# devitocodes/seigen

Hardware: AMD Instinct MI355X
Metric: M DoF-updates/sec, 3D elastic P=4 (higher is better)
Workload: dtype f64

## Files before the change

### seigen_amd/csrc/kernels_mfma.hip

```cpp
#include <hip/hip_runtime.h>

#include "kernels.hpp"

namespace sg {

template <typename R>
struct RT;
template <>
struct RT<double> {
  typedef double v4 __attribute__((ext_vector_type(4)));
  static constexpr bool SMALL = true;
  static __device__ __forceinline__ v4 big(double a, double b, v4 c) { return __builtin_amdgcn_mfma_f64_16x16x4f64(a, b, c, 0, 0, 0); }
  static __device__ __forceinline__ double small(double a, double b, double c) { return __builtin_amdgcn_mfma_f64_4x4x4f64(a, b, c, 0, 0, 0); }
};
template <>
struct RT<float> {
  typedef float v4 __attribute__((ext_vector_type(4)));
  static constexpr bool SMALL = false;
  static __device__ __forceinline__ v4 big(float a, float b, v4 c) { return __builtin_amdgcn_mfma_f32_16x16x4f32(a, b, c, 0, 0, 0); }
  static __device__ __forceinline__ float small(float, float, float c) { return c; }
};

template <typename R, int P>
constexpr int mfma_resident_blocks() {
  return sizeof(R) == 4 ? 3 : (P == 1 ? 4 : (P == 2 ? 3 : 2));
}

template <int P, typename R>
struct MG {
  static constexpr int ND = ElemDims<3, P>::ND;
  static constexpr int NF = ElemDims<3, P>::NF;
  static constexpr int KS = (ND + 3) / 4;
  static constexpr int KSF = (NF + 3) / 4;
  static constexpr int MTF = RT<R>::SMALL ? ND / 16 : (ND + 15) / 16;
  static constexpr int NSM = RT<R>::SMALL ? (ND % 16 + 3) / 4 : 0;
  static constexpr int MTT = MTF + NSM;
  static constexpr int MTFA = MTF > 0 ? MTF : 1;
  static constexpr int NSMA = NSM > 0 ? NSM : 1;
  static constexpr int S4 = (ND + 3) / 4;
  static constexpr int NFRAG_F = MTT * 3 * KS;
  static constexpr int NFRAG_G = 3 * MTT * KS;
  static constexpr int NFRAG_L = 4 * MTT * KSF;
  static constexpr int RK = (P >= 2) ? ElemDims<3, (P >= 2 ? P - 1 : 1)>::ND : 1;
  static constexpr int QLT = RK / 16;
  static constexpr int QST = (RK % 16 + 3) / 4;
  static constexpr int KR = (RK + 3) / 4;
  static constexpr int NFRAG_Q = (QLT + QST) * KS;
  static constexpr int NFRAG_P = 3 * MTT * KR;
};

template <typename R, int P, int FACT>
constexpr bool g_stash() {
  return sizeof(R) == 8 && P == 4 && FACT == 1;
}
template <int NOUT, int LT, int ST, int NKS>
struct CompactTiles {
  static constexpr int NL = NOUT * LT * NKS * 64, NS = NOUT * ST * NKS * 16, N = NL + NS;
  static constexpr int at(int o, int t, int ks) {
    return t < LT ? ((o * LT + t) * NKS + ks) * 64 : NL + ((o * ST + (t - LT)) * NKS + ks) * 16;
  }
};
constexpr int G_STASH_SLOTS = 36;
constexpr int G_STASH_WAVES = 8;
template <typename R, int P, int STASH>
struct GLds {
  using M = MG<P, R>;
  static constexpr int STW = 3 * G_STASH_SLOTS * 16;
  static constexpr int OFF_FO = ((int)sizeof(MeshDev) + 15) / 16 * 16;
  static constexpr int OFF_AV = OFF_FO + (STASH ? 64 * (int)sizeof(int) : 0);
  static constexpr int OFF_Q = OFF_AV + (int)sizeof(R) * (STASH ? CompactTiles<3, M::MTF, M::NSM, M::KR>::N : M::NFRAG_P * 64);
  static constexpr int OFF_AL = OFF_Q + (int)sizeof(R) * (STASH ? CompactTiles<1, M::QLT, M::QST, M::KS>::N : M::NFRAG_Q * 64);
  static constexpr int OFF_ST = OFF_AL + (int)sizeof(R) * (STASH ? CompactTiles<4, M::MTF, M::NSM, M::KSF>::N : M::NFRAG_L * 64);
  static constexpr int BYTES = OFF_ST + (STASH ? G_STASH_WAVES * STW * (int)sizeof(R) : 0);
};

#define LD_STREAM(p) __builtin_nontemporal_load(p)
#define ST_STREAM(p, v) __builtin_nontemporal_store((v), (p))
#define SG_PRIO(p) __builtin_amdgcn_s_setprio(p)
constexpr int SG_PRIO_F0 = 0x120, SG_PRIO_F1 = 0x320, SG_PRIO_F2 = 0x320, SG_PRIO_G0 = 0x120, SG_PRIO_G1 = 0x120;
#define SG_PRIO_VOL ((PRIO3 >> 8) & 3)
#define SG_PRIO_LIFT ((PRIO3 >> 4) & 3)
#define SG_PRIO_EPI (PRIO3 & 3)
#define MFMA64(a, b, c) RT<R>::big((a), (b), (c))
#define MFMA4(a, b, c) RT<R>::small((a), (b), (c))

#ifdef SG_STAMPS
#define STAMP(t)                                                                   \
  do {                                                                             \
    __builtin_amdgcn_sched_barrier(0);                                             \
    asm volatile("s_memtime %0\n\ts_waitcnt lgkmcnt(0)" : "=s"(t)::"memory");       \
    __builtin_amdgcn_sched_barrier(0);                                             \
  } while (0)
#define STAMP_DECL unsigned long long st0 = 0, st1 = 0, st2 = 0, st3 = 0, st4 = 0, sta = 0, stb = 0, sacc[4] = {0, 0, 0, 0}, ssub[3] = {0, 0, 0}, sitems = 0
#define STAMP_ACC                                                                  \
  do {                                                                             \
    sacc[0] += st1 - st0;                                                          \
    sacc[1] += st2 - st1;                                                          \
    sacc[2] += st3 - st2;                                                          \
    sacc[3] += st4 - st3;                                                          \
    if (sta) { ssub[0] += sta - st2; ssub[1] += stb - sta; ssub[2] += st3 - stb; } \
    sitems += 1;                                                                   \
  } while (0)
#define STAMP_FLUSH                                                                \
  do {                                                                             \
    if (A.dbg && lane == 0) {                                                      \
      for (int z = 0; z < 4; ++z) atomicAdd(&A.dbg[z], sacc[z]);                   \
      atomicAdd(&A.dbg[4], sitems);                                                \
      for (int z = 0; z < 3; ++z) atomicAdd(&A.dbg[5 + z], ssub[z]);               \
    }                                                                              \
  } while (0)
#else
#define STAMP(t) do { } while (0)
#define STAMP_DECL
#define STAMP_ACC do { } while (0)
#define STAMP_FLUSH do { } while (0)
#endif

template <int SYM, typename R>
__device__ __forceinline__ void load_tensor(const R* p, int stride, R (&T)[9]) {
  if (SYM) {
    T[0] = p[0];
    T[1] = p[1 * stride];
    T[2] = p[2 * stride];
    T[4] = p[4 * stride];
    T[5] = p[5 * stride];
    T[8] = p[8 * stride];
    T[3] = T[1];
    T[6] = T[2];
    T[7] = T[5];
  } else {
#pragma unroll
    for (int c = 0; c < 9; ++c) T[c] = p[c * stride];
  }
}
__device__ __forceinline__ constexpr bool upper(int ij) { return (ij / 3) <= (ij % 3); }

template <int SYM, int GHOST, typename R>
__device__ __forceinline__ void load_trace(const bool cube_face, const R* p, bool ghost, const int (&tl)[6], R (&T)[6]) {
  if (cube_face) {
    if (SYM) {
#pragma unroll
      for (int i = 0; i < 3; ++i) T[i] = p[GHOST ? (ghost ? i : tl[i]) : tl[i]];
    } else {
      const R* pa = p + ((GHOST && ghost) ? 0 : tl[0]);
#pragma unroll
      for (int i = 0; i < 3; ++i) T[i] = pa[GHOST ? (ghost ? i : i * 48) : i * 48];
    }
  } else if (SYM) {
    T[0] = p[0];
    T[1] = p[1 * 16];
    T[2] = p[2 * 16];
    T[3] = p[4 * 16];
    T[4] = p[5 * 16];
    T[5] = p[8 * 16];
  } else {
    const R *pa = p + tl[0], *pb = p + tl[3];
#pragma unroll
    for (int i = 0; i < 3; ++i) {
      T[i] = pa[i * 48];
      T[3 + i] = pb[i * 48];
    }
  }
}

__device__ __forceinline__ bool uniform_nonzero(double c) {
  return (__builtin_bit_cast(unsigned long long, c) << 1) != 0ull;
}
__device__ __forceinline__ bool uniform_nonzero(float c) { return (__builtin_bit_cast(unsigned, c) << 1) != 0u; }

struct LaneGeo {
  long c;
  int cc[3];
  bool valid;
  bool active;
};

typedef __attribute__((address_space(4))) const MfmaConst cMfmaConst;
typedef __attribute__((address_space(4))) const MfmaClassConst cMfmaClassConst;

template <typename MD>
__device__ __forceinline__ LaneGeo lane_geo(const MD& md, const StageArgs& A, long g, int w) {
  LaneGeo L;
  L.c = g * 16 + w;
  L.valid = L.c < md.ncube;
  const unsigned cl = L.valid ? (unsigned)L.c : 0u;
  const unsigned n0 = (unsigned)md.n[0], n1 = (unsigned)md.n[1];
  const unsigned t = cl / n0, z = t / n1;
  L.cc[0] = (int)(cl - t * n0);
  L.cc[1] = (int)(t - z * n1);
  L.cc[2] = (int)z;
  bool in = false;
  for (int bx = 0; bx < A.nbox; ++bx) {
    bool ib = true;
#pragma unroll
    for (int a = 0; a < 3; ++a) ib = ib && (L.cc[a] >= A.boxes_o[bx][a]) && (L.cc[a] < A.boxes_o[bx][a] + A.boxes_n[bx][a]);
    in = in || ib;
  }
  L.active = L.valid && in;
  return L;
}

template <typename R>
struct NbrRef {
  const R* p;
  int cstride;
  bool ghost;
  bool physical;
};

__device__ __forceinline__ LaneGeo lane_geo_all(long ncube, long g, int w) {
  LaneGeo L;
  L.c = g * 16 + w;
  L.valid = L.c < ncube;
  L.cc[0] = L.cc[1] = L.cc[2] = 0;
  L.active = L.valid;
  return L;
}

typedef int nbr4 __attribute__((ext_vector_type(4)));
__device__ __forceinline__ nbr4 load_nbr4(const StageArgs& A, long item, int w) {
  return *reinterpret_cast<const nbr4*>(A.nbr_tab + (item * 16 + w) * 4);
}
template <int ND, int NF, int NC, typename R_>
__device__ __forceinline__ NbrRef<R_> nbr_from_entry(const StageArgs& A, int e, int side, const R_* own_base) {
  NbrRef<R_> R;
  const R_* const fin = reinterpret_cast<const R_*>(A.in);
  R.cstride = 16;
  R.ghost = e < -1;
  R.physical = e == -1;
  const long slot = e < 0 ? 0 : e;
  const R_* pin = fin + ((slot >> 4) * (long)ND) * NC * 16 + (slot & 15);
  R.p = e < 0 ? own_base : pin;
  if (__any(R.ghost)) {
    if (R.ghost) {
      R.p = reinterpret_cast<const R_*>(A.ghost[side]) + (long)(-2 - e) * NF * 3;
      R.cstride = 1;
    }
  }
  return R;
}

struct ItemRange {
  long lo, hi, step;
  long chunk, xcd, nitems;
};
__device__ __forceinline__ ItemRange item_range(long nitems, int wave, int spread, long chunk) {
  ItemRange r;
  const long wpb = blockDim.x >> 6;
  r.chunk = 0;
  r.xcd = 0;
  r.nitems = nitems;
  if (spread) {
    r.lo = (long)blockIdx.x * wpb + wave;
    r.hi = nitems;
    r.step = (long)gridDim.x * wpb;
    return r;
  }
  const long nblk = gridDim.x;
  const long xcd = blockIdx.x % 8;
  const long slot = blockIdx.x / 8;
  const long blocks_here = (nblk - xcd + 7) / 8;
  r.step = blocks_here * wpb;
  if (chunk > 0) {
    const long nchunks = (nitems + chunk - 1) / chunk;
    const long mine = (nchunks - xcd + 7) / 8;
    r.chunk = chunk;
    r.xcd = xcd;
    r.lo = slot * wpb + wave;
    r.hi = mine > 0 ? mine * chunk : 0;
    return r;
  }
  const long ipx = (nitems + 7) / 8;
  r.lo = xcd * ipx + slot * wpb + wave;
  r.hi = (xcd + 1) * ipx < nitems ? (xcd + 1) * ipx : nitems;
  return r;
}
__device__ __forceinline__ long item_of(const ItemRange& r, long it) {
  if (r.chunk == 0) return it;
  const long c = it / r.chunk;
  const long item = (c * 8 + r.xcd) * r.chunk + (it - c * r.chunk);
  return item < r.nitems ? item : -1;
}

template <int N, typename R, int NT = 256>
__device__ __forceinline__ void copy_to_lds(R* dst, const R* __restrict__ src) {
  constexpr int PER = (N + NT - 1) / NT;
  R v[PER];
#pragma unroll
  for (int j = 0; j < PER; ++j) {
    const int i = threadIdx.x + j * NT;
    v[j] = (i < N) ? src[i] : R(0);
  }
#pragma unroll
  for (int j = 0; j < PER; ++j) {
    const int i = threadIdx.x + j * NT;
    if (i < N) dst[i] = v[j];
  }
}

template <typename CT, int NOUT, int LT, int ST, int NKS, typename R, int NT>
__device__ __forceinline__ void copy_compact(R* dst, const R* __restrict__ src) {
  constexpr int PER = (CT::N + NT - 1) / NT;
  R v[PER];
#pragma unroll
  for (int j = 0; j < PER; ++j) {
    const int i = threadIdx.x + j * NT;
    int s = 0;
    if (i < CT::NL) {
      const int fr = i >> 6, o = fr / (LT * NKS), rem = fr - o * (LT * NKS);
      s = (o * (LT + ST) * NKS + rem) * 64 + (i & 63);
    } else {
      const int i2 = i - CT::NL, fr = i2 >> 4, c = i2 & 15, o = fr / (ST * NKS), rem = fr - o * (ST * NKS);
      s = (o * (LT + ST) * NKS + LT * NKS + rem) * 64 + (c & 3) + 16 * (c >> 2);
    }
    v[j] = (i < CT::N) ? src[s] : R(0);
  }
#pragma unroll
  for (int j = 0; j < PER; ++j) {
    const int i = threadIdx.x + j * NT;
    if (i < CT::N) dst[i] = v[j];
  }
}

template <int NV, int NL, typename R, int NT = 256>
__device__ __forceinline__ void load_tables(R* sAV, R* sAL, const StageArgs& A) {
  copy_to_lds<NV * 64, R, NT>(sAV, reinterpret_cast<const R*>(A.fragV));
  copy_to_lds<NL * 64, R, NT>(sAL, reinterpret_cast<const R*>(A.fragL));
  __syncthreads();
}

template <int NV, int NL, typename R>
__device__ __forceinline__ void load_tables(R* sAV, R* sAL, MeshDev* sMd, const StageArgs& A) {
  const int* src = reinterpret_cast<const int*>(A.md);
  int* dst = reinterpret_cast<int*>(sMd);
  constexpr int NI = (int)(sizeof(MeshDev) / sizeof(int)), PERI = (NI + 255) / 256;
  int w[PERI];
#pragma unroll
  for (int j = 0; j < PERI; ++j) {
    const int i = threadIdx.x + j * 256;
    w[j] = (i < NI) ? src[i] : 0;
  }
  copy_to_lds<NV * 64>(sAV, reinterpret_cast<const R*>(A.fragV));
  copy_to_lds<NL * 64>(sAL, reinterpret_cast<const R*>(A.fragL));
#pragma unroll
  for (int j = 0; j < PERI; ++j) {
    const int i = threadIdx.x + j * 256;
    if (i < NI) dst[i] = w[j];
  }
  __syncthreads();
}


template <typename R>
__device__ __forceinline__ R ndot(R c0, R c1, R c2, R t0, R t1, R t2) {
  R r = c0 * t0;
  r = __builtin_fma(c1, t1, r);
  r = __builtin_fma(c2, t2, r);
  return r;
}
template <>
__device__ __forceinline__ float ndot<float>(float c0, float c1, float c2, float t0, float t1, float t2) {
  float r = c0 * t0;
  r = __builtin_fmaf(c1, t1, r);
  r = __builtin_fmaf(c2, t2, r);
  return r;
}
__device__ __forceinline__ double fma_of(double a, double b, double c) { return __builtin_fma(a, b, c); }
__device__ __forceinline__ float fma_of(float a, float b, float c) { return __builtin_fmaf(a, b, c); }

template <int SYM, typename R>
__device__ __forceinline__ R trace_flux(const bool cube_face, int i, R wf, const R (&cnf)[3], const R (&tc)[2], const R (&T)[6]) {
  if (cube_face) return wf * (tc[0] * T[i]);
  if (SYM) {
    const int s0 = i, s1 = i == 0 ? 1 : (i == 1 ? 3 : 4), s2 = i == 0 ? 2 : (i == 1 ? 4 : 5);
    return wf * ndot<R>(cnf[0], cnf[1], cnf[2], T[s0], T[s1], T[s2]);
  }
  const R r = tc[0] * T[i];
  return wf * fma_of(tc[1], T[3 + i], r);
}


template <typename R, int P, int MODE, int SYM, bool FACT, bool STASH, bool DYN>
__device__ __forceinline__ void stage_G_body(const StageArgs& A) {
  using M = MG<P, R>;
  constexpr int NT = STASH ? 512 : 256;
  typedef typename RT<R>::v4 d4;
  constexpr int PRIO3 = MODE ? SG_PRIO_G1 : SG_PRIO_G0;
  constexpr int ND = M::ND, NF = M::NF, KS = M::KS, KSF = M::KSF, MTF = M::MTF, NSM = M::NSM, MTT = M::MTT, S4 = M::S4;
  constexpr int PF = sizeof(R) == 4 ? 6 : 4;
  constexpr int QLT = M::QLT, QST = M::QST, KR = M::KR;
  using CP = CompactTiles<3, MTF, NSM, KR>;
  using CQ = CompactTiles<1, QLT, QST, KS>;
  using CL = CompactTiles<4, MTF, NSM, KSF>;
  using LY = GLds<R, P, STASH>;
  constexpr int STW = LY::STW;
  R *sAV = nullptr, *sQ = nullptr, *sAL = nullptr, *sSt = nullptr;
  MeshDev* sMdp = nullptr;
  int* sFo = nullptr;
  if constexpr (DYN) {
    extern __shared__ __attribute__((aligned(16))) unsigned char sg_dyn_lds[];
    sMdp = reinterpret_cast<MeshDev*>(sg_dyn_lds);
    sFo = reinterpret_cast<int*>(sg_dyn_lds + LY::OFF_FO);
    sAV = reinterpret_cast<R*>(sg_dyn_lds + LY::OFF_AV);
    sQ = reinterpret_cast<R*>(sg_dyn_lds + LY::OFF_Q);
    sAL = reinterpret_cast<R*>(sg_dyn_lds + LY::OFF_AL);
    sSt = reinterpret_cast<R*>(sg_dyn_lds + LY::OFF_ST);
  } else {
    __shared__ R sAV_[(FACT ? M::NFRAG_P : M::NFRAG_G) * 64];
    __shared__ R sQ_[FACT ? M::NFRAG_Q * 64 : 1];
    __shared__ R sAL_[M::NFRAG_L * 64];
    __shared__ MeshDev sMd_;
    sAV = sAV_, sQ = sQ_, sAL = sAL_, sMdp = &sMd_;
  }
  MeshDev& sMd = *sMdp;
  if constexpr (STASH) {
    static_assert(ND <= G_STASH_SLOTS && 4 * KS <= G_STASH_SLOTS, "a stash slot per B row of the Q pass");
    copy_to_lds<(int)(sizeof(MeshDev) / sizeof(int)), int, NT>(reinterpret_cast<int*>(&sMd), reinterpret_cast<const int*>(A.md));
    copy_compact<CQ, 1, QLT, QST, KS, R, NT>(sQ, reinterpret_cast<const R*>(A.fragQ));
    copy_compact<CP, 3, MTF, NSM, KR, R, NT>(sAV, reinterpret_cast<const R*>(A.fragV));
    copy_compact<CL, 4, MTF, NSM, KSF, R, NT>(sAL, reinterpret_cast<const R*>(A.fragL));
    if (threadIdx.x < 64) {
      const int f = threadIdx.x >> 4, bq4 = 4 * (threadIdx.x & 3) + ((threadIdx.x >> 2) & 3);
      sFo[threadIdx.x] = (int)A.md->fnode[f][bq4 < NF ? bq4 : 0] * 16 * (int)sizeof(R);
    }
    __syncthreads();
  } else {
    if constexpr (FACT) copy_to_lds<M::NFRAG_Q * 64>(sQ, reinterpret_cast<const R*>(A.fragQ));
    load_tables<(FACT ? M::NFRAG_P : M::NFRAG_G), M::NFRAG_L>(sAV, sAL, &sMd, A);
  }

  const int lane = threadIdx.x & 63;
  const int wave = __builtin_amdgcn_readfirstlane(threadIdx.x >> 6);
  const int q = lane >> 4, w = lane & 15;
  typedef __attribute__((address_space(4))) const MeshDev cMeshDev;
  const cMeshDev* md = (const cMeshDev*)(unsigned long long)A.md;
  const R* __restrict__ in = reinterpret_cast<const R*>(A.in);
  R* __restrict__ out = reinterpret_cast<R*>(A.out);
  const R c_self = (R)A.c_self, c_new = (R)A.c_new;
  const long ngroups = sMd.ncube_pad >> 4;
  const ItemRange ir = item_range(A.item_list ? (long)A.nlist : ngroups * 6, wave, A.spread, A.order_chunk);

  STAMP_DECL;
  for (long it = ir.lo; it < ir.hi; it += ir.step) {
    STAMP(st0);
    const long iti = item_of(ir, it);
    if (iti < 0) continue;
    const long item = A.item_list ? (long)A.item_list[iti] : iti;
    const long g = item / 6;
    const int k = (int)(item - g * 6);
    const LaneGeo L = A.all_active ? lane_geo_all(sMd.ncube, g, w) : lane_geo(sMd, A, g, w);
    const nbr4 nbe = load_nbr4(A, item, w);
    if (!__any(L.active)) continue;
    const R* own = in + ((g * 6 + k) * (long)ND) * 3 * 16 + w;
    int qo = q * 3 * 16;
    asm volatile("" : "+v"(qo));
    const R* ownq = own + qo;
    const R* ownl = (4 * (KS - 1) + q < ND) ? ownq + (KS - 1) * 4 * 3 * 16 : own;
    auto brow = [&](int ks) { return (ks == KS - 1) ? ownl : ownq + ks * 4 * 3 * 16; };
    int lo = lane;
    asm volatile("" : "+v"(lo));
    const int lo4 = (lo & 3) + ((lo >> 4) << 2);
    R* const stw = sSt + (STASH ? wave * STW : 0) + lo;
    const char* const str = reinterpret_cast<const char*>(sSt + (STASH ? wave * STW : 0) + (lo & 15));
    auto tile = [&](const R* tab, int full, int at, int t, int nlarge) { return STASH ? tab[at + (t < nlarge ? lo : lo4)] : tab[full * 64 + lo]; };

    R Jm[3][3], cnf[4][3];
#pragma unroll
    for (int r = 0; r < 3; ++r)
#pragma unroll
      for (int j = 0; j < 3; ++j) Jm[r][j] = (R)(-md->Jinv[k][r][j]);
#pragma unroll
    for (int f = 0; f < 4; ++f)
#pragma unroll
      for (int j = 0; j < 3; ++j) cnf[f][j] = (R)md->cn[k][f][j];

    R Sd[3][S4], So[3][S4];
#pragma unroll
    for (int i = 0; i < 3; ++i)
#pragma unroll
      for (int m = 0; m < S4; ++m) Sd[i][m] = So[i][m] = R(0);

    constexpr int NB = 2;
    constexpr int NBO = (FACT && !STASH) ? NB : 1;
    R nx[NB][KSF][3], nxo[NBO][KSF][3];
    auto request = [&](int f, R (&dst)[KSF][3], R (&dso)[KSF][3]) {
      const NbrRef<R> NR = nbr_from_entry<ND, NF, 3>(A, nbe[f], 2 * sMd.nb_axis[k][f] + (sMd.nb_dir[k][f] > 0 ? 1 : 0), own);
#pragma unroll
      for (int ks = 0; ks < KSF; ++ks) {
        const int bb = (4 * ks + q < NF) ? 4 * ks + q : 0;
        const int on = sMd.fnode[f][bb];
        const int nn = NR.ghost ? sMd.nb_fnode[k][f][bb] : (NR.physical ? on : sMd.nb_node[k][f][bb]);
#pragma unroll
        for (int i = 0; i < 3; ++i) {
          dst[ks][i] = NR.p[(nn * 3 + i) * NR.cstride];
          if constexpr (FACT && !STASH) dso[ks][i] = own[(on * 3 + i) * 16];
        }
      }
    };
    SG_PRIO(SG_PRIO_VOL);
    STAMP(st1);
    auto fold_dir = [&](int r, const d4 (&acc)[M::MTFA][3], const R (&accs)[M::NSMA][3]) {
#pragma unroll
      for (int kk = 0; kk < 3; ++kk) {
        const R c = Jm[r][kk];
        if (uniform_nonzero(c)) {
#pragma unroll
          for (int i = 0; i < 3; ++i) {
#pragma unroll
            for (int t = 0; t < MTF; ++t)
#pragma unroll
              for (int reg = 0; reg < 4; ++reg) {
                if (4 * t + reg >= S4) continue;
                if (i == kk)
                  Sd[i][4 * t + reg] += c * acc[t][i][reg];
                else
                  So[i + kk - 1][4 * t + reg] += c * acc[t][i][reg];
              }
#pragma unroll
            for (int t = 0; t < NSM; ++t) {
              if (i == kk)
                Sd[i][4 * MTF + t] += c * accs[t][i];
              else
                So[i + kk - 1][4 * MTF + t] += c * accs[t][i];
            }
          }
        }
      }
#pragma unroll
      for (int m = 0; m < S4; ++m)
#pragma unroll
        for (int i = 0; i < 3; ++i) asm volatile("" : "+v"(Sd[i][m]), "+v"(So[i][m]));
    };
    auto tiles_step = [&](int nks, int r, int ks, const R (&b)[3], d4 (&acc)[M::MTFA][3], R (&accs)[M::NSMA][3]) {
#pragma unroll
      for (int t = 0; t < MTT; ++t) {
        const R a = tile(sAV, (r * MTT + t) * nks + ks, CP::at(r, t, ks), t, MTF);
#pragma unroll
        for (int i = 0; i < 3; ++i) {
          if (t < MTF)
            acc[t < MTF ? t : 0][i] = MFMA64(a, b[i], acc[t < MTF ? t : 0][i]);
          else
            accs[t < MTF ? 0 : t - MTF][i] = MFMA4(a, b[i], accs[t < MTF ? 0 : t - MTF][i]);
        }
      }
    };
    auto clear_acc = [&](d4 (&acc)[M::MTFA][3], R (&accs)[M::NSMA][3]) {
#pragma unroll
      for (int i = 0; i < 3; ++i) {
#pragma unroll
        for (int t = 0; t < MTF; ++t) acc[t][i] = d4{0, 0, 0, 0};
#pragma unroll
        for (int t = 0; t < NSM; ++t) accs[t][i] = R(0);
      }
    };
    if constexpr (!FACT) {
      constexpr int NS = 3 * KS;
      R bq[PF][3];
#pragma unroll
      for (int s = 0; s < PF; ++s)
#pragma unroll
        for (int i = 0; i < 3; ++i) bq[s][i] = brow(s % KS)[i * 16];
#pragma unroll
      for (int r = 0; r < 3; ++r) {
        d4 acc[M::MTFA][3];
        R accs[M::NSMA][3];
        clear_acc(acc, accs);
#pragma unroll
        for (int ks = 0; ks < KS; ++ks) {
          const int s = r * KS + ks;
          R b[3];
#pragma unroll
          for (int i = 0; i < 3; ++i) b[i] = bq[s % PF][i];
          if (s + PF < NS) {
#pragma unroll
            for (int i = 0; i < 3; ++i) bq[s % PF][i] = brow((s + PF) % KS)[i * 16];
          }
          tiles_step(KS, r, ks, b, acc, accs);
        }
        fold_dir(r, acc, accs);
      }
    } else {
      d4 yl[QLT > 0 ? QLT : 1][3];
      R ys[QST > 0 ? QST : 1][3];
#pragma unroll
      for (int i = 0; i < 3; ++i) {
#pragma unroll
        for (int t = 0; t < QLT; ++t) yl[t][i] = d4{0, 0, 0, 0};
#pragma unroll
        for (int t = 0; t < QST; ++t) ys[t][i] = R(0);
      }
      R bq[PF][3];
#pragma unroll
      for (int s = 0; s < PF && s < KS; ++s)
#pragma unroll
        for (int i = 0; i < 3; ++i) bq[s][i] = brow(s)[i * 16];
#pragma unroll
      for (int ks = 0; ks < KS; ++ks) {
        R b[3];
#pragma unroll
        for (int i = 0; i < 3; ++i) b[i] = bq[ks % PF][i];
        if (ks + PF < KS) {
#pragma unroll
          for (int i = 0; i < 3; ++i) bq[ks % PF][i] = brow(ks + PF)[i * 16];
        }
        if constexpr (STASH) {
#pragma unroll
          for (int i = 0; i < 3; ++i) stw[(i * G_STASH_SLOTS + 4 * ks) * 16] = b[i];
        }
#pragma unroll
        for (int t = 0; t < QLT + QST; ++t) {
          const R a = tile(sQ, t * KS + ks, CQ::at(0, t, ks), t, QLT);
#pragma unroll
          for (int i = 0; i < 3; ++i) {
            if (t < QLT)
              yl[t < QLT ? t : 0][i] = MFMA64(a, b[i], yl[t < QLT ? t : 0][i]);
            else
              ys[t < QLT ? 0 : t - QLT][i] = MFMA4(a, b[i], ys[t < QLT ? 0 : t - QLT][i]);
          }
        }
      }
#pragma unroll
      for (int r = 0; r < 3; ++r) {
        d4 acc[M::MTFA][3];
        R accs[M::NSMA][3];
        clear_acc(acc, accs);
#pragma unroll
        for (int ks = 0; ks < KR; ++ks) {
          R b[3];
#pragma unroll
          for (int i = 0; i < 3; ++i) b[i] = (ks < 4 * QLT) ? yl[(ks / 4) < QLT ? ks / 4 : 0][i][ks % 4] : ys[(ks - 4 * QLT) >= 0 && (ks - 4 * QLT) < QST ? ks - 4 * QLT : 0][i];
          tiles_step(KR, r, ks, b, acc, accs);
        }
        fold_dir(r, acc, accs);
      }
    }

    STAMP(st2);
    {
#pragma unroll
      for (int f0 = 0; f0 < NB - 1; ++f0) request(f0, nx[f0], nxo[f0 % NBO]);
      SG_PRIO(SG_PRIO_LIFT);
#pragma unroll
      for (int f = 0; f < 4; ++f) {
        R(&flf)[KSF][3] = nx[f % NB];
        if constexpr (STASH) {
          const nbr4 fo = *reinterpret_cast<const nbr4*>(&sFo[f * 16 + (lo >> 4) * 4]);
#pragma unroll
          for (int ks = 0; ks < KSF; ++ks)
#pragma unroll
            for (int i = 0; i < 3; ++i)
              flf[ks][i] += *reinterpret_cast<const R*>(str + fo[ks] + i * G_STASH_SLOTS * 16 * (int)sizeof(R));
        } else if constexpr (FACT) {
#pragma unroll
          for (int ks = 0; ks < KSF; ++ks)
#pragma unroll
            for (int i = 0; i < 3; ++i) flf[ks][i] += nxo[f % NBO][ks][i];
        }
#pragma unroll
        for (int t = 0; t < MTT; ++t) {
          if (t == 0 && f + NB - 1 < 4) request(f + NB - 1, nx[(f + NB - 1) % NB], nxo[(f + NB - 1) % NBO]);
          auto fold = [&](int m0, int nm, const R (&v)[3][4]) {
#pragma unroll
            for (int kk = 0; kk < 3; ++kk) {
              const R c = cnf[f][kk];
              if (uniform_nonzero(c)) {
#pragma unroll
                for (int i = 0; i < 3; ++i)
#pragma unroll
                  for (int j = 0; j < 4; ++j)
                    if (j < nm && m0 + j < S4) {
                      if (i == kk)
                        Sd[i][m0 + j] += c * v[i][j];
                      else
                        So[i + kk - 1][m0 + j] += c * v[i][j];
                    }
              }
            }
#pragma unroll
            for (int j = 0; j < 4; ++j)
              if (j < nm && m0 + j < S4) {
#pragma unroll
                for (int i = 0; i < 3; ++i) asm volatile("" : "+v"(Sd[i][m0 + j]), "+v"(So[i][m0 + j]));
              }
          };
          if (t < MTF) {
            d4 tmp[3];
#pragma unroll
            for (int i = 0; i < 3; ++i) tmp[i] = d4{0, 0, 0, 0};
#pragma unroll
            for (int ks = 0; ks < KSF; ++ks) {
              const R a = tile(sAL, (f * MTT + t) * KSF + ks, CL::at(f, t, ks), t, MTF);
#pragma unroll
              for (int i = 0; i < 3; ++i) tmp[i] = MFMA64(a, flf[ks][i], tmp[i]);
            }
            {
              R v[3][4];
#pragma unroll
              for (int i = 0; i < 3; ++i)
#pragma unroll
                for (int reg = 0; reg < 4; ++reg) v[i][reg] = tmp[i][reg];
              fold(4 * t, 4, v);
            }
          } else {
            R tmp[3] = {R(0), R(0), R(0)};
#pragma unroll
            for (int ks = 0; ks < KSF; ++ks) {
              const R a = tile(sAL, (f * MTT + t) * KSF + ks, CL::at(f, t, ks), t, MTF);
#pragma unroll
              for (int i = 0; i < 3; ++i) tmp[i] = MFMA4(a, flf[ks][i], tmp[i]);
            }
            {
              const R v[3][4] = {{tmp[0], 0, 0, 0}, {tmp[1], 0, 0, 0}, {tmp[2], 0, 0, 0}};
              fold(4 * MTF + (t - MTF), 1, v);
            }
          }
        }
      }
    }

    SG_PRIO(SG_PRIO_EPI);
    STAMP(st3);
    {
      const long e = (L.valid ? L.c : 0) * 6 + k;
      const R lam = (R)(A.per_cell ? A.lam[e] : A.lam0);
      const R mu = (R)(A.per_cell ? A.mu[e] : A.mu0);
      const long obase = ((g * 6 + k) * (long)ND) * 9 * 16 + w;
      int qo9 = q * 9 * 16;
      asm volatile("" : "+v"(qo9));
      const long ob_q = obase + qo9;
      const long ob_l = (4 * (S4 - 1) + q < ND) ? ob_q + (long)(S4 - 1) * 4 * 9 * 16 : obase;
      auto orow = [&](int m) { return (m == S4 - 1) ? ob_l : ob_q + (long)m * 4 * 9 * 16; };
      if constexpr (SYM || MODE == 0) {
        constexpr int NL = SYM ? 6 : 9;
        constexpr int PDE = 4;
        R po[PDE][6];
        auto line = [](int c) { return SYM ? (c < 3 ? c : (c < 5 ? c + 1 : 8)) : c; };
        auto fetch_old = [&](int m) {
          const long o1 = orow(m);
#pragma unroll
          for (int c = 0; c < 6; ++c) po[m % PDE][c] = LD_STREAM(&out[o1 + line(c) * 16]);
        };
        if (MODE == 1) {
#pragma unroll
          for (int m = 0; m < PDE && m < S4; ++m) fetch_old(m);
        }
#pragma unroll
        for (int m = 0; m < S4; ++m) {
          const R tr = lam * (Sd[0][m] + Sd[1][m] + Sd[2][m]);
#pragma unroll
          for (int i = 0; i < 3; ++i) {
            Sd[i][m] = R(2) * mu * Sd[i][m] + tr;
            So[i][m] = mu * So[i][m];
          }
          if (MODE == 1) {
            Sd[0][m] = c_self * po[m % PDE][0] + c_new * Sd[0][m];
            So[0][m] = c_self * po[m % PDE][1] + c_new * So[0][m];
            So[1][m] = c_self * po[m % PDE][2] + c_new * So[1][m];
            Sd[1][m] = c_self * po[m % PDE][3] + c_new * Sd[1][m];
            So[2][m] = c_self * po[m % PDE][4] + c_new * So[2][m];
            Sd[2][m] = c_self * po[m % PDE][5] + c_new * Sd[2][m];
            if (m + PDE < S4) fetch_old(m + PDE);
          }
#pragma unroll
          for (int i = 0; i < 3; ++i) asm volatile("" : "+v"(Sd[i][m]), "+v"(So[i][m]));
        }
#pragma unroll
        for (int m = 0; m < S4; ++m) {
          const int a = 4 * m + q;
          const long o = orow(m);
          if (L.active && a < ND) {
            ST_STREAM(&out[o + 0 * 16], Sd[0][m]);
            ST_STREAM(&out[o + 1 * 16], So[0][m]);
            ST_STREAM(&out[o + 2 * 16], So[1][m]);
            ST_STREAM(&out[o + 4 * 16], Sd[1][m]);
            ST_STREAM(&out[o + 5 * 16], So[2][m]);
            ST_STREAM(&out[o + 8 * 16], Sd[2][m]);
            if (!SYM) {
              ST_STREAM(&out[o + 3 * 16], So[0][m]);
              ST_STREAM(&out[o + 6 * 16], So[1][m]);
              ST_STREAM(&out[o + 7 * 16], So[2][m]);
            }
          }
        }
        (void)NL;
      } else {
#pragma unroll
        for (int m = 0; m < S4; ++m) {
          const int a = 4 * m + q;
          const long o = orow(m);
          const R tr = lam * (Sd[0][m] + Sd[1][m] + Sd[2][m]);
          R s[9];
          s[0] = R(2) * mu * Sd[0][m] + tr;
          s[4] = R(2) * mu * Sd[1][m] + tr;
          s[8] = R(2) * mu * Sd[2][m] + tr;
          s[1] = s[3] = mu * So[0][m];
          s[2] = s[6] = mu * So[1][m];
          s[5] = s[7] = mu * So[2][m];
#pragma unroll
          for (int ij = 0; ij < 9; ++ij) s[ij] = c_self * out[o + ij * 16] + c_new * s[ij];
          if (L.active && a < ND) {
#pragma unroll
            for (int ij = 0; ij < 9; ++ij) out[o + ij * 16] = s[ij];
          }
        }
      }
    }
    STAMP(st4);
    STAMP_ACC;
  }
  STAMP_FLUSH;
}

template <typename R, int P, int MODE, int SYM, int FACT>
__global__ __launch_bounds__((g_stash<R, P, FACT>() ? 512 : 256), (g_stash<R, P, FACT>() ? 1 : mfma_resident_blocks<R, P>())) void mfma_stage_G(StageArgs A) {
  if constexpr (g_stash<R, P, FACT>()) {
    if (blockDim.x == 512)
      stage_G_body<R, P, MODE, SYM, true, true, true>(A);
    else
      stage_G_body<R, P, MODE, SYM, true, false, true>(A);
  } else {
    stage_G_body<R, P, MODE, SYM, FACT != 0, false, false>(A);
  }
}

template <typename R, int P, int MODE, int SYM, int GHOST>
__global__ __launch_bounds__(256, (mfma_resident_blocks<R, P>())) void mfma_stage_F(StageArgs A) {
  using M = MG<P, R>;
  typedef typename RT<R>::v4 d4;
  constexpr int PRIO3 = MODE == 1 ? SG_PRIO_F1 : (MODE == 2 ? SG_PRIO_F2 : SG_PRIO_F0);
  constexpr int ND = M::ND, NF = M::NF, KS = M::KS, KSF = M::KSF, MTF = M::MTF, NSM = M::NSM, MTT = M::MTT;
  __shared__ R sAV[M::NFRAG_F * 64];
  __shared__ R sAL[M::NFRAG_L * 64];
  __shared__ nbr4 sFt[3 * 6 * 4 * 4];
  {
    const nbr4* src = reinterpret_cast<const nbr4*>(A.ftab);
    for (int i = threadIdx.x; i < 3 * 6 * 4 * 4; i += 256) sFt[i] = src[i];
  }
  load_tables<M::NFRAG_F, M::NFRAG_L>(sAV, sAL, A);
  const cMfmaConst& mk = *(const cMfmaConst*)(unsigned long long)A.mk;

  const int lane = threadIdx.x & 63;
  const int wave = __builtin_amdgcn_readfirstlane(threadIdx.x >> 6);
  const int q = lane >> 4, w = lane & 15;
  typedef __attribute__((address_space(4))) const MeshDev cMeshDev;
  const cMeshDev* md = (const cMeshDev*)(unsigned long long)A.md;
  const R* __restrict__ in = reinterpret_cast<const R*>(A.in);
  const R* __restrict__ aux = reinterpret_cast<const R*>(A.aux);
  R* __restrict__ out = reinterpret_cast<R*>(A.out);
  const R c_self = (R)A.c_self, c_aux = (R)A.c_aux, c_new = (R)A.c_new;
  const long ngroups = mk.ncube_pad >> 4;
  const ItemRange ir = item_range(A.item_list ? (long)A.nlist : ngroups * 6, wave, A.spread, A.order_chunk);

  STAMP_DECL;
  for (long it = ir.lo; it < ir.hi; it += ir.step) {
    STAMP(st0);
    const long iti = item_of(ir, it);
    if (iti < 0) continue;
    const long item = A.item_list ? (long)A.item_list[iti] : iti;
    const long g = item / 6;
    const int k = (int)(item - g * 6);
    const LaneGeo L = A.all_active ? lane_geo_all(mk.ncube, g, w) : lane_geo(mk, A, g, w);
    const cMfmaClassConst& kc = mk.cls[k];
    const nbr4 nbe = load_nbr4(A, item, w);
    if (!__any(L.active)) continue;
    const R* own = in + ((g * 6 + k) * (long)ND) * 9 * 16 + w;
    int qo = q * 9 * 16;
    asm volatile("" : "+v"(qo));
    const R* ownq = own + qo;
    const R* ownl = (4 * (KS - 1) + q < ND) ? ownq + (KS - 1) * 4 * 9 * 16 : own;
    auto brow = [&](int ks) { return (ks == KS - 1) ? ownl : ownq + ks * 4 * 9 * 16; };
    int lo = lane;
    asm volatile("" : "+v"(lo));

    R Jm[3][3], cnf[4][3];
#pragma unroll
    for (int r = 0; r < 3; ++r)
#pragma unroll
      for (int j = 0; j < 3; ++j) Jm[r][j] = (R)md->Jinv[k][r][j];
#pragma unroll
    for (int f = 0; f < 4; ++f)
#pragma unroll
      for (int j = 0; j < 3; ++j) cnf[f][j] = (R)md->cn[k][f][j];

    d4 acc[3][M::MTFA];
    R accs[3][M::NSMA];
    const long e = (L.valid ? L.c : 0) * 6 + k;
    const long ubase = ((g * 6 + k) * (long)ND) * 3 * 16 + w;
    int qo3 = q * 3 * 16;
    asm volatile("" : "+v"(qo3));
    const long ub_q = ubase + qo3;
    constexpr bool FUSED = MODE >= 1, SELF = MODE == 1;
    const bool early = FUSED && sizeof(R) == 8 && uniform_nonzero(c_new);
    R cs = c_self, ca = c_aux, cn = c_new;
    if (MODE == 1 && A.rho2 != nullptr) {
      cs = (R)A.rho2[2 * e];
      ca *= (R)A.rho2[2 * e + 1];
      cn *= (R)A.rho2[2 * e + 1];
    }
    R sig = (R)0;
    bool sig_folded = false;
    if (FUSED && A.sponge_sigma != nullptr && L.active) {
      sig = (R)A.sponge_sigma[e];
      if (sig == sig && sig != (R)0) {
        if (SELF && A.uabs == A.out) {
          cs -= cn * sig;
          sig_folded = true;
        } else if (A.uabs == A.aux) {
          ca -= cn * sig;
          sig_folded = true;
        }
      }
    }
    R po[M::MTFA][4][3], pa[M::MTFA][4][3], pos[M::NSMA][3], pas[M::NSMA][3];
    auto fetch_old = [&]() {
#pragma unroll
      for (int t = 0; t < MTF; ++t)
#pragma unroll
        for (int reg = 0; reg < 4; ++reg) {
          const bool row_ok = RT<R>::SMALL || (16 * t + 4 * reg + q < ND);
          const long o = row_ok ? ub_q + (long)(16 * t + 4 * reg) * 3 * 16 : ubase;
#pragma unroll
          for (int i = 0; i < 3; ++i) {
            po[t][reg][i] = SELF ? LD_STREAM(&out[o + i * 16]) : R(0);
            pa[t][reg][i] = LD_STREAM(&aux[o + i * 16]);
          }
        }
#pragma unroll
      for (int t = 0; t < NSM; ++t) {
        const int a = 16 * MTF + 4 * t + q;
        const long o = (a < ND) ? ub_q + (long)(16 * MTF + 4 * t) * 3 * 16 : ubase;
#pragma unroll
        for (int i = 0; i < 3; ++i) {
          pos[t][i] = SELF ? LD_STREAM(&out[o + i * 16]) : R(0);
          pas[t][i] = LD_STREAM(&aux[o + i * 16]);
        }
      }
    };
    if (early) {
      fetch_old();
      const R icn = R(1) / cn;
#pragma unroll
      for (int t = 0; t < MTF; ++t)
#pragma unroll
        for (int reg = 0; reg < 4; ++reg)
#pragma unroll
          for (int i = 0; i < 3; ++i) acc[i][t][reg] = SELF ? (cs * po[t][reg][i] + ca * pa[t][reg][i]) * icn : (ca * pa[t][reg][i]) * icn;
#pragma unroll
      for (int t = 0; t < NSM; ++t)
#pragma unroll
        for (int i = 0; i < 3; ++i) accs[i][t] = SELF ? (cs * pos[t][i] + ca * pas[t][i]) * icn : (ca * pas[t][i]) * icn;
    } else {
#pragma unroll
      for (int i = 0; i < 3; ++i) {
#pragma unroll
        for (int t = 0; t < MTF; ++t) acc[i][t] = d4{0, 0, 0, 0};
#pragma unroll
        for (int t = 0; t < NSM; ++t) accs[i][t] = R(0);
      }
    }

    SG_PRIO(SG_PRIO_VOL);
    STAMP(st1);
    auto do_volume = [&]() {
      {
        constexpr int PFV = sizeof(R) == 4 ? 2 : 1;
        R Tq[PFV][9];
#pragma unroll
        for (int s0 = 0; s0 < PFV && s0 < KS; ++s0) load_tensor<SYM>(brow(s0), 16, Tq[s0]);
#pragma unroll
        for (int ks = 0; ks < KS; ++ks) {
          R T[9];
#pragma unroll
          for (int c = 0; c < 9; ++c) T[c] = Tq[ks % PFV][c];
          if (ks + PFV < KS) {
            load_tensor<SYM>(brow(ks + PFV), 16, Tq[ks % PFV]);
          }
#pragma unroll
          for (int r = 0; r < 3; ++r) {
            R Tt[3];
#pragma unroll
            for (int i = 0; i < 3; ++i) Tt[i] = Jm[r][0] * T[i * 3 + 0] + Jm[r][1] * T[i * 3 + 1] + Jm[r][2] * T[i * 3 + 2];
#pragma unroll
            for (int t = 0; t < MTT; ++t) {
              const R a = sAV[(t * 3 * KS + KS * r + ks) * 64 + lo];
#pragma unroll
              for (int i = 0; i < 3; ++i) {
                if (t < MTF)
                  acc[i][t < MTF ? t : 0] = MFMA64(a, Tt[i], acc[i][t < MTF ? t : 0]);
                else
                  accs[i][t < MTF ? 0 : t - MTF] = MFMA4(a, Tt[i], accs[i][t < MTF ? 0 : t - MTF]);
              }
            }
          }
        }
      }

    };
    auto do_lifts = [&]() {
      constexpr int PFL = sizeof(R) == 4 ? 3 : 2;
      const R* np[4];
      R wf[4];
      int noff[4][KSF];
      bool gh[4];
      int tl[4][6];
      R tc[4][2];
#pragma unroll
      for (int f = 0; f < 4; ++f) {
        const NbrRef<R> NR = nbr_from_entry<ND, NF, 9>(A, nbe[f], 2 * kc.nb_axis[f] + (kc.nb_dir[f] > 0 ? 1 : 0), own);
        np[f] = NR.p;
        gh[f] = GHOST && NR.ghost;
#pragma unroll
        for (int c = 0; c < 6; ++c) tl[f][c] = kc.tr_line[SYM ? 1 : 0][f][c];
        tc[f][0] = (R)kc.tr_cn[f][0];
        tc[f][1] = (R)kc.tr_cn[f][1];
        wf[f] = NR.physical ? R(-1) : R(1);
        const int var = NR.ghost ? 1 : (NR.physical ? 2 : 0);
        const nbr4 o4 = sFt[((var * 6 + k) * 4 + f) * 4 + q];
#pragma unroll
        for (int ks = 0; ks < KSF; ++ks) noff[f][ks] = o4[ks];
      }
      R nq[PFL][6];
      auto cube_face = [](int f) { return f == 0 || f == 3; };
      STAMP(sta);
      {
        constexpr int NS = 4 * KSF;
#pragma unroll
        for (int s = 0; s < PFL; ++s)
          load_trace<SYM, GHOST>(cube_face(s / KSF), np[s / KSF] + noff[s / KSF][s % KSF], gh[s / KSF], tl[s / KSF], nq[s]);
#pragma unroll
        for (int f = 0; f < 4; ++f) {
          if (f == 1) STAMP(stb);
#pragma unroll
          for (int ks = 0; ks < KSF; ++ks) {
            const int s = f * KSF + ks;
            R fl[3];
#pragma unroll
            for (int i = 0; i < 3; ++i)
              fl[i] = trace_flux<SYM>(cube_face(f), i, wf[f], cnf[f], tc[f], nq[s % PFL]);
            if (s + PFL < NS) {
              const int f1 = (s + PFL) / KSF, k1 = (s + PFL) % KSF;
              load_trace<SYM, GHOST>(cube_face(f1), np[f1] + noff[f1][k1], gh[f1], tl[f1], nq[s % PFL]);
            }
#pragma unroll
            for (int t = 0; t < MTT; ++t) {
              const R a = sAL[((f * MTT + t) * KSF + ks) * 64 + lo];
#pragma unroll
              for (int i = 0; i < 3; ++i) {
                if (t < MTF)
                  acc[i][t < MTF ? t : 0] = MFMA64(a, fl[i], acc[i][t < MTF ? t : 0]);
                else
                  accs[i][t < MTF ? 0 : t - MTF] = MFMA4(a, fl[i], accs[i][t < MTF ? 0 : t - MTF]);
              }
            }
          }
        }
      }

    };
    do_volume();
    STAMP(st2);
    SG_PRIO(SG_PRIO_LIFT);
    do_lifts();

    SG_PRIO(SG_PRIO_EPI);
    STAMP(st3);
    if (A.sponge_sigma != nullptr) {
      if (!FUSED && L.active) sig = (R)A.sponge_sigma[e];
      int slot = -1;
      if (sig != sig) slot = A.sponge_slot[e];
      const bool sp_here = sig != (R)0 && !sig_folded;
      if (__any(sp_here)) {
        if (sp_here) {
          constexpr int NR = 4 * MTF + NSM;
          const bool dense = slot >= 0;
          const R* pb = dense ? reinterpret_cast<const R*>(A.sponge_pre) + ((long)(slot >> 4) * ND * 3 + q * 3) * 16 + (slot & 15)
                              : reinterpret_cast<const R*>(A.uabs) + ub_q;
          constexpr int es = 16;
          const R sc = dense ? (R)1 : sig;
          R uo[NR][3];
#pragma unroll
          for (int r = 0; r < NR; ++r) {
            const int o = (4 * r + q < ND) ? 4 * r * 3 * es : 0;
#pragma unroll
            for (int i = 0; i < 3; ++i) uo[r][i] = pb[o + i * es];
          }
#pragma unroll
          for (int r = 0; r < NR; ++r)
// ... 235 lines not shown
```

Measured before the change: 92170.

## Fold elastic constitutive law and old-value blend into gradient accumulation for MODE 1

For MODE 1 with P=4 (or P=3 in f64), the lam/mu constitutive scaling and the c_new factor are folded into the fold coefficients, so the stress is built directly while gradients accumulate. The old output values are loaded early, during the first direction's k-steps, and seed the accumulators after scaling by c_self. This removes the separate epilogue stress transform and hides the load latency of the old values behind MFMA work. In exchange it adds more FMAs per fold term because the trace contributions go to three diagonals, keeps the accumulators live for longer, and changes how the non-symmetric lower entries are stored, using a corrected difference of upper and lower old values.

```diff
diff --git a/seigen_amd/csrc/kernels_mfma.hip b/seigen_amd/csrc/kernels_mfma.hip
--- a/seigen_amd/csrc/kernels_mfma.hip
+++ b/seigen_amd/csrc/kernels_mfma.hip
@@ -52,6 +52,10 @@
 template <typename R, int P, int FACT>
 constexpr bool g_stash() {
   return sizeof(R) == 8 && P == 4 && FACT == 1;
+}
+template <typename R, int P>
+constexpr bool g_early() {
+  return P == 4 || (P == 3 && sizeof(R) == 8);
 }
 template <int NOUT, int LT, int ST, int NKS>
 struct CompactTiles {
@@ -387,6 +391,7 @@
   typedef typename RT<R>::v4 d4;
   constexpr int PRIO3 = MODE ? SG_PRIO_G1 : SG_PRIO_G0;
   constexpr int ND = M::ND, NF = M::NF, KS = M::KS, KSF = M::KSF, MTF = M::MTF, NSM = M::NSM, MTT = M::MTT, S4 = M::S4;
+  constexpr bool EARLY = MODE == 1 && g_early<R, P>();
   constexpr int PF = sizeof(R) == 4 ? 6 : 4;
   constexpr int QLT = M::QLT, QST = M::QST, KR = M::KR;
   using CP = CompactTiles<3, MTF, NSM, KR>;
@@ -431,7 +436,6 @@
 
   const int lane = threadIdx.x & 63;
   const int wave = __builtin_amdgcn_readfirstlane(threadIdx.x >> 6);
-  const int q = lane >> 4, w = lane & 15;
   typedef __attribute__((address_space(4))) const MeshDev cMeshDev;
   const cMeshDev* md = (const cMeshDev*)(unsigned long long)A.md;
   const R* __restrict__ in = reinterpret_cast<const R*>(A.in);
@@ -448,6 +452,9 @@
     const long item = A.item_list ? (long)A.item_list[iti] : iti;
     const long g = item / 6;
     const int k = (int)(item - g * 6);
+    int ln = lane;
+    if constexpr (EARLY) asm volatile("" : "+v"(ln));
+    const int q = ln >> 4, w = ln & 15;
     const LaneGeo L = A.all_active ? lane_geo_all(sMd.ncube, g, w) : lane_geo(sMd, A, g, w);
     const nbr4 nbe = load_nbr4(A, item, w);
     if (!__any(L.active)) continue;
@@ -475,10 +482,71 @@
       for (int j = 0; j < 3; ++j) cnf[f][j] = (R)md->cn[k][f][j];
 
     R Sd[3][S4], So[3][S4];
-#pragma unroll
-    for (int i = 0; i < 3; ++i)
-#pragma unroll
-      for (int m = 0; m < S4; ++m) Sd[i][m] = So[i][m] = R(0);
+    auto out_rows = [&](long& obase, long& ob_q, long& ob_l) {
+      int wo = w, qo9 = q * 9 * 16;
+      if constexpr (EARLY) asm volatile("" : "+v"(wo));
+      asm volatile("" : "+v"(qo9));
+      obase = ((g * 6 + k) * (long)ND) * 9 * 16 + wo;
+      ob_q = obase + qo9;
+      ob_l = (4 * (S4 - 1) + q < ND) ? ob_q + (long)(S4 - 1) * 4 * 9 * 16 : obase;
+    };
+    R cmu = R(0), cla = R(0);
+    long eo_b = 0, eo_q = 0, eo_l = 0;
+    if constexpr (EARLY) {
+      const long e = (L.valid ? L.c : 0) * 6 + k;
+      cmu = (R)(A.per_cell ? A.mu[e] : A.mu0);
+      cla = (R)(A.per_cell ? A.lam[e] : A.lam0);
+      out_rows(eo_b, eo_q, eo_l);
+    } else {
+#pragma unroll
+      for (int i = 0; i < 3; ++i)
+#pragma unroll
+        for (int m = 0; m < S4; ++m) Sd[i][m] = So[i][m] = R(0);
+    }
+    auto fetch_old = [&](int m) {
+      const long o1 = (m == S4 - 1) ? eo_l : eo_q + (long)m * 4 * 9 * 16;
+      Sd[0][m] = LD_STREAM(&out[o1 + 0 * 16]);
+      So[0][m] = LD_STREAM(&out[o1 + 1 * 16]);
+      So[1][m] = LD_STREAM(&out[o1 + 2 * 16]);
+      Sd[1][m] = LD_STREAM(&out[o1 + 4 * 16]);
+      So[2][m] = LD_STREAM(&out[o1 + 5 * 16]);
+      Sd[2][m] = LD_STREAM(&out[o1 + 8 * 16]);
+    };
+    static_assert(S4 == KS, "a row-quad of old values per k-step");
+    auto old_at_step = [&](int ks) {
+      if constexpr (EARLY) fetch_old(ks);
+    };
+    auto seed_scale = [&]() {
+      __builtin_amdgcn_sched_barrier(0);
+      cmu = c_new * cmu;
+      cla = c_new * cla;
+#pragma unroll
+      for (int m = 0; m < S4; ++m)
+#pragma unroll
+        for (int i = 0; i < 3; ++i) {
+          Sd[i][m] = c_self * Sd[i][m];
+          So[i][m] = c_self * So[i][m];
+        }
+    };
+    auto coefs = [&](R c, R& cd, R& cl, R& co) {
+      cd = cl = co = c;
+      if constexpr (EARLY) {
+        co = c * cmu;
+        cl = c * cla;
+        cd = R(2) * co + cl;
+      }
+    };
+    auto fold_term = [&](int kk, int i, int m, R cd, R cl, R co, R a) {
+      if (i == kk) {
+        Sd[i][m] += cd * a;
+        if constexpr (EARLY) {
+          Sd[(i + 1) % 3][m] += cl * a;
+          Sd[(i + 2) % 3][m] += cl * a;
+        }
+      } else {
+        So[i + kk - 1][m] += co * a;
+      }
+    };
 
     constexpr int NB = 2;
     constexpr int NBO = (FACT && !STASH) ? NB : 1;
@@ -504,6 +572,8 @@
       for (int kk = 0; kk < 3; ++kk) {
         const R c = Jm[r][kk];
         if (uniform_nonzero(c)) {
+          R cd, cl, co;
+          coefs(c, cd, cl, co);
 #pragma unroll
           for (int i = 0; i < 3; ++i) {
 #pragma unroll
@@ -511,18 +581,10 @@
 #pragma unroll
               for (int reg = 0; reg < 4; ++reg) {
                 if (4 * t + reg >= S4) continue;
-                if (i == kk)
-                  Sd[i][4 * t + reg] += c * acc[t][i][reg];
-                else
-                  So[i + kk - 1][4 * t + reg] += c * acc[t][i][reg];
+                fold_term(kk, i, 4 * t + reg, cd, cl, co, acc[t][i][reg]);
               }
 #pragma unroll
-            for (int t = 0; t < NSM; ++t) {
-              if (i == kk)
-                Sd[i][4 * MTF + t] += c * accs[t][i];
-              else
-                So[i + kk - 1][4 * MTF + t] += c * accs[t][i];
-            }
+            for (int t = 0; t < NSM; ++t) fold_term(kk, i, 4 * MTF + t, cd, cl, co, accs[t][i]);
           }
         }
       }
@@ -575,7 +637,11 @@
 #pragma unroll
             for (int i = 0; i < 3; ++i) bq[s % PF][i] = brow((s + PF) % KS)[i * 16];
           }
+          if (r == 0) old_at_step(ks);
           tiles_step(KS, r, ks, b, acc, accs);
+        }
+        if constexpr (EARLY) {
+          if (r == 0) seed_scale();
         }
         fold_dir(r, acc, accs);
       }
@@ -603,6 +669,7 @@
 #pragma unroll
           for (int i = 0; i < 3; ++i) bq[ks % PF][i] = brow(ks + PF)[i * 16];
         }
+        old_at_step(ks);
         if constexpr (STASH) {
 #pragma unroll
           for (int i = 0; i < 3; ++i) stw[(i * G_STASH_SLOTS + 4 * ks) * 16] = b[i];
@@ -631,6 +698,9 @@
           for (int i = 0; i < 3; ++i) b[i] = (ks < 4 * QLT) ? yl[(ks / 4) < QLT ? ks / 4 : 0][i][ks % 4] : ys[(ks - 4 * QLT) >= 0 && (ks - 4 * QLT) < QST ? ks - 4 * QLT : 0][i];
           tiles_step(KR, r, ks, b, acc, accs);
         }
+        if constexpr (EARLY) {
+          if (r == 0) seed_scale();
+        }
         fold_dir(r, acc, accs);
       }
     }
@@ -664,16 +734,13 @@
             for (int kk = 0; kk < 3; ++kk) {
               const R c = cnf[f][kk];
               if (uniform_nonzero(c)) {
+                R cd, cl, co;
+                coefs(c, cd, cl, co);
 #pragma unroll
                 for (int i = 0; i < 3; ++i)
 #pragma unroll
                   for (int j = 0; j < 4; ++j)
-                    if (j < nm && m0 + j < S4) {
-                      if (i == kk)
-                        Sd[i][m0 + j] += c * v[i][j];
-                      else
-                        So[i + kk - 1][m0 + j] += c * v[i][j];
-                    }
+                    if (j < nm && m0 + j < S4) fold_term(kk, i, m0 + j, cd, cl, co, v[i][j]);
               }
             }
 #pragma unroll
@@ -722,47 +789,69 @@
     STAMP(st3);
     {
       const long e = (L.valid ? L.c : 0) * 6 + k;
-      const R lam = (R)(A.per_cell ? A.lam[e] : A.lam0);
-      const R mu = (R)(A.per_cell ? A.mu[e] : A.mu0);
-      const long obase = ((g * 6 + k) * (long)ND) * 9 * 16 + w;
-      int qo9 = q * 9 * 16;
-      asm volatile("" : "+v"(qo9));
-      const long ob_q = obase + qo9;
-      const long ob_l = (4 * (S4 - 1) + q < ND) ? ob_q + (long)(S4 - 1) * 4 * 9 * 16 : obase;
+      const R lam = EARLY ? R(0) : (R)(A.per_cell ? A.lam[e] : A.lam0);
+      const R mu = EARLY ? R(0) : (R)(A.per_cell ? A.mu[e] : A.mu0);
+      long obase, ob_q, ob_l;
+      out_rows(obase, ob_q, ob_l);
       auto orow = [&](int m) { return (m == S4 - 1) ? ob_l : ob_q + (long)m * 4 * 9 * 16; };
-      if constexpr (SYM || MODE == 0) {
-        constexpr int NL = SYM ? 6 : 9;
-        constexpr int PDE = 4;
-        R po[PDE][6];
-        auto line = [](int c) { return SYM ? (c < 3 ? c : (c < 5 ? c + 1 : 8)) : c; };
-        auto fetch_old = [&](int m) {
-          const long o1 = orow(m);
-#pragma unroll
-          for (int c = 0; c < 6; ++c) po[m % PDE][c] = LD_STREAM(&out[o1 + line(c) * 16]);
-        };
-        if (MODE == 1) {
-#pragma unroll
-          for (int m = 0; m < PDE && m < S4; ++m) fetch_old(m);
-        }
-#pragma unroll
-        for (int m = 0; m < S4; ++m) {
-          const R tr = lam * (Sd[0][m] + Sd[1][m] + Sd[2][m]);
-#pragma unroll
-          for (int i = 0; i < 3; ++i) {
-            Sd[i][m] = R(2) * mu * Sd[i][m] + tr;
-            So[i][m] = mu * So[i][m];
-          }
+      if constexpr (SYM || MODE == 0 || EARLY) {
+        if constexpr (!EARLY) {
+          constexpr int PDE = 4;
+          R po[PDE][6];
+          auto line = [](int c) { return SYM ? (c < 3 ? c : (c < 5 ? c + 1 : 8)) : c; };
+          auto fetch_late = [&](int m) {
+            const long o1 = orow(m);
+#pragma unroll
+            for (int c = 0; c < 6; ++c) po[m % PDE][c] = LD_STREAM(&out[o1 + line(c) * 16]);
+          };
           if (MODE == 1) {
-            Sd[0][m] = c_self * po[m % PDE][0] + c_new * Sd[0][m];
-            So[0][m] = c_self * po[m % PDE][1] + c_new * So[0][m];
-            So[1][m] = c_self * po[m % PDE][2] + c_new * So[1][m];
-            Sd[1][m] = c_self * po[m % PDE][3] + c_new * Sd[1][m];
-            So[2][m] = c_self * po[m % PDE][4] + c_new * So[2][m];
-            Sd[2][m] = c_self * po[m % PDE][5] + c_new * Sd[2][m];
-            if (m + PDE < S4) fetch_old(m + PDE);
-          }
-#pragma unroll
-          for (int i = 0; i < 3; ++i) asm volatile("" : "+v"(Sd[i][m]), "+v"(So[i][m]));
+#pragma unroll
+            for (int m = 0; m < PDE && m < S4; ++m) fetch_late(m);
+          }
+#pragma unroll
+          for (int m = 0; m < S4; ++m) {
+            const R tr = lam * (Sd[0][m] + Sd[1][m] + Sd[2][m]);
+#pragma unroll
+            for (int i = 0; i < 3; ++i) {
+              Sd[i][m] = R(2) * mu * Sd[i][m] + tr;
+              So[i][m] = mu * So[i][m];
+            }
+            if (MODE == 1) {
+              Sd[0][m] = c_self * po[m % PDE][0] + c_new * Sd[0][m];
+              So[0][m] = c_self * po[m % PDE][1] + c_new * So[0][m];
+              So[1][m] = c_self * po[m % PDE][2] + c_new * So[1][m];
+              Sd[1][m] = c_self * po[m % PDE][3] + c_new * Sd[1][m];
+              So[2][m] = c_self * po[m % PDE][4] + c_new * So[2][m];
+              Sd[2][m] = c_self * po[m % PDE][5] + c_new * Sd[2][m];
+              if (m + PDE < S4) fetch_late(m + PDE);
+            }
+#pragma unroll
+            for (int i = 0; i < 3; ++i) asm volatile("" : "+v"(Sd[i][m]), "+v"(So[i][m]));
+          }
+        }
+        R lw[3][S4];
+        if constexpr (EARLY && !SYM) {
+          constexpr int PDE = 4;
+          R pu[PDE][3], pl[PDE][3];
+          auto fetch_pair = [&](int m) {
+            const long o1 = orow(m);
+            pu[m % PDE][0] = LD_STREAM(&out[o1 + 1 * 16]);
+            pu[m % PDE][1] = LD_STREAM(&out[o1 + 2 * 16]);
+            pu[m % PDE][2] = LD_STREAM(&out[o1 + 5 * 16]);
+            pl[m % PDE][0] = LD_STREAM(&out[o1 + 3 * 16]);
+            pl[m % PDE][1] = LD_STREAM(&out[o1 + 6 * 16]);
+            pl[m % PDE][2] = LD_STREAM(&out[o1 + 7 * 16]);
+          };
+#pragma unroll
+          for (int m = 0; m < PDE && m < S4; ++m) fetch_pair(m);
+#pragma unroll
+          for (int m = 0; m < S4; ++m) {
+#pragma unroll
+            for (int j = 0; j < 3; ++j) lw[j][m] = fma_of(c_self, pl[m % PDE][j] - pu[m % PDE][j], So[j][m]);
+            if (m + PDE < S4) fetch_pair(m + PDE);
+#pragma unroll
+            for (int j = 0; j < 3; ++j) asm volatile("" : "+v"(lw[j][m]));
+          }
         }
 #pragma unroll
         for (int m = 0; m < S4; ++m) {
@@ -776,13 +865,13 @@
             ST_STREAM(&out[o + 5 * 16], So[2][m]);
             ST_STREAM(&out[o + 8 * 16], Sd[2][m]);
             if (!SYM) {
-              ST_STREAM(&out[o + 3 * 16], So[0][m]);
-              ST_STREAM(&out[o + 6 * 16], So[1][m]);
-              ST_STREAM(&out[o + 7 * 16], So[2][m]);
+              ST_STREAM(&out[o + 3 * 16], EARLY ? lw[0][m] : So[0][m]);
+              ST_STREAM(&out[o + 6 * 16], EARLY ? lw[1][m] : So[1][m]);
+              ST_STREAM(&out[o + 7 * 16], EARLY ? lw[2][m] : So[2][m]);
             }
           }
         }
-        (void)NL;
+        (void)lam, (void)mu;
       } else {
 #pragma unroll
         for (int m = 0; m < S4; ++m) {
```

Result: no change. 92710 (median of 6 runs) (+0.6%).
